# wangty537/raft_optical_flow

Hardware: AMD Instinct MI355X
Metric: image-pairs/s at Sintel 436x1024, 32 iters; corr-lookup GB/s vs HBM peak (higher is better)
Workload: dtype fp32 (convs: f16x3 split MFMA, fp32 accumulate); 1 GPU; RAFT-full inference, 436x1024 padded to 440x1024, 1 pair(s)/GPU/step, iters=32, all-pairs corr, hipGraph; global_batch=1, parallelism=frame-pair sharding x1

## Files before the change

include/raft_hip.h:

```cpp
#ifndef RAFT_HIP_H_
#define RAFT_HIP_H_

#include <stddef.h>

#ifdef __cplusplus
extern "C" {
#endif

#define RAFT_HIP_ABI_VERSION 19

#define RAFT_E_INVALID (-1)
#define RAFT_E_ALIGN (-2)

typedef void* raft_stream_t;

int raft_hip_abi_version(void);
const char* raft_hip_arch(void);
const char* raft_hip_last_error(void);
const char* raft_hip_source_hash(void);
int raft_debug_launch_span(int enable);
int raft_debug_launch_span_read(unsigned long long* host, int n);
int raft_debug_fill_lds_nan(raft_stream_t stream);

size_t raft_corr_pyramid_floats(int B, int H, int W, int num_levels);
// ... 82 lines not shown
typedef struct raft_conv2d_params {
  const float* in0; int in0_ld; int in0_c;
  const float* in1; int in1_ld; int in1_c;
  int batch, in_h, in_w;
  int out_h, out_w;
  int kh, kw, stride_h, stride_w, pad_h, pad_w;
  int mode;
  const float* weight;
  const float* bias;
  int n;
  float* out; int out_ld;
  int epilogue; float alpha; int split;
  const float* aux0; int aux0_ld;
  const float* aux1; int aux1_ld;
  float* out1; int out1_ld;
  const float* add0; int add0_ld;
  int precision;
  int* range_flag;
  float* stats_part; int stats_ld;
  const float* in_norm; int in_norm_relu;
  const void* weight_s;
} raft_conv2d_params;

#define RAFT_RANGE_LIMIT 32768.0f

int raft_conv2d_stats_slots(const raft_conv2d_params* p);
int raft_conv2d_halo_tile_rows(const raft_conv2d_params* p);
int raft_conv2d_halo_tiles_per_wg(const raft_conv2d_params* p);
#define RAFT_CONV_KERNEL_HALO 1
#define RAFT_CONV_KERNEL_GEMM 2
#define RAFT_CONV_KERNEL_STEM 3
#define RAFT_CONV_KERNEL_SMALLN 4
#define RAFT_CONV_KERNEL_SMALLN3X3 5
struct raft_conv2d_form {
  int kernel;
  int tile_rows;
  int tile_cols;
  int tiles_per_wg;
  int loader_waves;
  int compute_waves_per_simd;
  int gemm_k_groups;
  int smalln_tile_rows;
};
int raft_conv2d_form(const raft_conv2d_params* p, struct raft_conv2d_form* out);
int raft_conv2d_pair_form(const raft_conv2d_params* p0, const raft_conv2d_params* p1,
                          struct raft_conv2d_form out[2], int* one_launch);
int raft_conv2d_in_norm_ok(const raft_conv2d_params* p);
int raft_instnorm_merge(const float* part, int slots_per_image, int B, int C, int stats_ld, float eps,
                        float* stats, raft_stream_t stream);
size_t raft_instnorm_merge_ws_floats(int slots_per_image, int B, int C);
int raft_instnorm_merge_ws(const float* part, int slots_per_image, int B, int C, int stats_ld, float eps, void* ws,
                           float* stats, raft_stream_t stream);
size_t raft_instnorm_merge_counters(int B, int C);
int raft_instnorm_merge_fused(const float* part, int slots_per_image, int B, int C, int stats_ld, float eps, void* ws,
                              int* counters, float* stats, raft_stream_t stream);

int raft_conv2d_packed_shape(int mode, int n, int kh, int kw, int cin, int* n_pad, int* k_pad);
int raft_conv2d(const raft_conv2d_params* p, raft_stream_t stream);
int raft_conv2d_pair(const raft_conv2d_params* p0, const raft_conv2d_params* p1, raft_stream_t stream);
int raft_conv2d_set_halo_loaders(int nl);
int raft_conv2d_set_halo_ks(int ks);
int raft_conv2d_split_weight(const float* w, void* out, int n_pad, int k_pad, raft_stream_t stream);
size_t raft_conv2d_split_scaled_bytes(int n_pad, int k_pad);
int raft_conv2d_split_weight_scaled(const float* w, void* out, int n_pad, int k_pad, raft_stream_t stream);
int raft_conv2d_split_weight_prec(const float* w, void* out, int n_pad, int k_pad, int precision,
                                  raft_stream_t stream);
// ... 69 lines not shown
```

raft_optical_flow_amd/_lib.py:

```python
from __future__ import annotations

import ctypes
import os
import threading

_HERE = os.path.dirname(os.path.abspath(__file__))
LIB_PATH = os.environ.get("RAFT_HIP_LIB") or os.path.join(_HERE, "libraft_hip.so")

c_int = ctypes.c_int
c_float = ctypes.c_float
c_size_t = ctypes.c_size_t
c_long = ctypes.c_long
c_void_p = ctypes.c_void_p
c_char_p = ctypes.c_char_p
P = c_void_p

RAFT_CONV_VEC = 0
RAFT_CONV_GATHER = 1

PREC_FP32 = 0
PREC_F16X3 = 1
PREC_F16 = 2
PREC_BF16 = 3
PRECISIONS = {"fp32": PREC_FP32, "f16x3": PREC_F16X3, "f16": PREC_F16, "bf16": PREC_BF16}
# ... 25 lines not shown
        ("batch", c_int), ("in_h", c_int), ("in_w", c_int),
        ("out_h", c_int), ("out_w", c_int),
        ("kh", c_int), ("kw", c_int), ("stride_h", c_int), ("stride_w", c_int), ("pad_h", c_int), ("pad_w", c_int),
        ("mode", c_int),
        ("weight", P), ("bias", P),
        ("n", c_int),
        ("out", P), ("out_ld", c_int),
        ("epilogue", c_int), ("alpha", c_float), ("split", c_int),
        ("aux0", P), ("aux0_ld", c_int),
        ("aux1", P), ("aux1_ld", c_int),
        ("out1", P), ("out1_ld", c_int),
        ("add0", P), ("add0_ld", c_int),
        ("precision", c_int),
        ("range_flag", P),
        ("stats_part", P), ("stats_ld", c_int),
        ("in_norm", P), ("in_norm_relu", c_int),
        ("weight_s", P),
    ]


CARRY_MAX_SEGS = 8


class Copy2D(ctypes.Structure):

    _fields_ = [("src", P), ("src_ld", c_long), ("dst", P), ("dst_ld", c_long), ("rows", c_long), ("cols", c_long)]


CONV_KERNEL_HALO = 1
CONV_KERNEL_GEMM = 2
CONV_KERNEL_STEM = 3
CONV_KERNEL_SMALLN = 4
CONV_KERNEL_SMALLN3X3 = 5


class ConvForm(ctypes.Structure):

    _fields_ = [
        ("kernel", c_int), ("tile_rows", c_int), ("tile_cols", c_int), ("tiles_per_wg", c_int),
        ("loader_waves", c_int), ("compute_waves_per_simd", c_int), ("gemm_k_groups", c_int),
        ("smalln_tile_rows", c_int),
    ]

    def astuple(self):
        return tuple(getattr(self, f) for f, _ in self._fields_)


def conv_form(p: ConvParams) -> ConvForm:
    f = ConvForm()
    call("raft_conv2d_form", ctypes.byref(p), ctypes.byref(f))
    return f


def conv_pair_form(p0: ConvParams, p1: ConvParams):
    f = (ConvForm * 2)()
    one = c_int(0)
    call("raft_conv2d_pair_form", ctypes.byref(p0), ctypes.byref(p1), f, ctypes.byref(one))
    return f[0], f[1], bool(one.value)


_PROTOS = {
    "raft_hip_abi_version": (c_int, []),
    "raft_hip_arch": (c_char_p, []),
    "raft_hip_last_error": (c_char_p, []),
    "raft_hip_source_hash": (c_char_p, []),
    "raft_debug_fill_lds_nan": (c_int, [P]),
# ... 151 lines not shown
```

raft_optical_flow_amd/csrc/conv_halo.hip:

```cpp
#include <atomic>
#include <type_traits>

#include "conv_common.hpp"

namespace raft {
namespace {

constexpr int HTW = 16;
constexpr int HTH = 8;
constexpr int HTH_BIG = 16;
constexpr int HALO_LDS = 160 * 1024;

struct HaloArgs {
  raft_conv2d_params p;
  const float* inv_scale;
  int K;
  int nch;
  int nk;
  int gn;
  int tx_n, ty_n;
  unsigned w_bytes, in0_bytes, in1_bytes;
};

struct HaloLaunch {
  HaloArgs a[2];
  int sp0, sp1;
  int m;
  int grid0;
};

constexpr int patch_slots(int T, int U, int D, int late = 0) {
  for (int pa = 1; pa < 16; ++pa) {
    bool ok = true;
    for (int c = pa; c < 512 && ok; ++c) {
      const int last = (c - pa) * T + T - 1;
      const int rd = last == 0 ? -1 : (last - 1) / U;
      ok = (c * T) / U - D > rd + late;
    }
    if (ok) return pa;
  }
  return 16;
}
constexpr int halo_lds_bytes(int T, int U, int D, int BNT, int PI, int WR) {
  return U * (D + 1) * BNT * WR + patch_slots(T, U, D) * PI * 1024;
}

template <int KH, int KW, int BNT, int WR = 128, int TH = HTH>
struct HaloCfg {
  static constexpr int T = KH * KW;
  static constexpr int U = (BNT == 32 && T > 1) ? 4 : 2;
  static constexpr int LB = HALO_LDS;
  static constexpr int PH = TH + KH - 1, PW = HTW + KW - 1, NPIX = PH * PW;
  static constexpr int PI = (NPIX + 7) / 8;
#ifdef HALO_D
  static constexpr int D = halo_lds_bytes(T, U, HALO_D, BNT, PI, WR) <= LB   ? HALO_D
                           : halo_lds_bytes(T, U, 3, BNT, PI, WR) <= LB ? 3
                                                                              : 2;
#else
  static constexpr int D = halo_lds_bytes(T, U, 3, BNT, PI, WR) <= LB ? 3 : 2;
#endif
  static constexpr int PA = patch_slots(T, U, D);
#ifndef HALO_WX
#define HALO_WX 0
#endif
  static constexpr int DW = (T > 1 && D == 3 && HALO_WX > 0 &&
                             U * (D + HALO_WX + 1) * BNT * WR + PA * PI * 1024 + 16 * 1024 <= LB)
                                ? D + HALO_WX
                                : D;
  static constexpr int SB = U * (DW + 1);
  static constexpr int LDS_B = SB * BNT * WR, LDS_A = PA * PI * 1024;
};

#ifdef STAMPS
__device__ unsigned long long g_hstamp[8 * 16384];
__device__ unsigned long long g_lstamp[8 * 16384];
__device__ __forceinline__ unsigned long long hstamp_real() {
  unsigned long long t;
  __builtin_amdgcn_sched_barrier(0);
  asm volatile("s_memrealtime %0\n\ts_waitcnt lgkmcnt(0)" : "=s"(t)::"memory");
  __builtin_amdgcn_sched_barrier(0);
  return t;
}
__device__ __forceinline__ unsigned long long hstamp_now() {
  unsigned long long t;
  __builtin_amdgcn_sched_barrier(0);
  asm volatile("s_memtime %0\n\ts_waitcnt lgkmcnt(0)" : "=s"(t)::"memory");
  __builtin_amdgcn_sched_barrier(0);
  return t;
}
#endif

constexpr int gcd_c(int a, int b) { return b == 0 ? a : gcd_c(b, a % b); }
__host__ __device__ inline int halo_nkp(int nk, int U, int T, bool multi) {
  const int l = multi ? U / gcd_c(U, T) * T : U;
  return cdiv(nk, l) * l;
}
template <int KH, int KW, int BNT, int PREC, bool ENC>
constexpr int halo_norm_bytes(int LDS_B, int LDS_A, int D) {
  return (ENC && KH == 3 && KW == 3 && D == 3) ? ((HALO_LDS - LDS_B - LDS_A) & ~1023) : 0;
}

template <int KH, int KW, int BNT, int PREC, bool ENC = false, int TH = HTH, bool MT = false, int NL = 4, int KS = 1>
__device__ __forceinline__ void halo_body(const HaloArgs* args, int prob, int nt, int st0, int ntl_arg, char* smem) {
  constexpr bool X3 = PREC == RAFT_PREC_F16X3;
  constexpr bool BF = PREC == RAFT_PREC_BF16;
  using C = HaloCfg<KH, KW, BNT, X3 ? 128 : 64, TH>;
  constexpr int T = C::T, U = C::U, D = C::D, PW = C::PW, NPIX = C::NPIX, PI = C::PI, PA = C::PA, SB = C::SB;
  constexpr int DW = C::DW;
  constexpr int WROW = X3 ? 128 : 64;
  constexpr int QPR = WROW / 16;
  constexpr int RPP = 1024 / WROW;
  constexpr int NBI = BNT / RPP;
  constexpr int NWP = U * NBI / NL;
#ifndef HALO_KSW
#define HALO_KSW 0
#endif
  constexpr bool KSW = KS > 1 && HALO_KSW;
  constexpr int NWPC = KSW ? U * NBI / (4 * KS) : 1;
  constexpr int LNWP = KSW ? 0 : NWP;
  constexpr int WN = BNT == 128 ? 2 : 1;
  constexpr int WVM = 4 / WN;
  constexpr int MF = TH / 2 / WVM;
  constexpr int WCOL = BNT / WN;
  constexpr int NSUB = WCOL / 32;
  constexpr bool SC = X3 && TH == HTH_BIG;
  static_assert(MF >= 1 && MF * WVM * 2 == TH, "tile rows");
  static_assert(!(X3 && MF > 1) || SC, "f16x3 2 x 2 blocks need the one-accumulator (scaled) form");
  static_assert(!ENC || WN == 1, "the InstanceNorm partials are per 32-pixel block of all columns");

#ifndef HALO_NOLSPLIT
#define HALO_NOLSPLIT 0
#endif
  constexpr bool LSPLIT = T > 1 && D == 3 && !(HALO_NOLSPLIT && !ENC);
#ifndef HALO_SGB
#define HALO_SGB 1
#endif
  constexpr int SGB = (ENC && NL == 8) ? 0 : HALO_SGB;
#ifndef HALO_RELAX
#define HALO_RELAX 1
#endif
  constexpr int NRD1 = NSUB * 2 * (X3 ? 2 : 1) + MF * 2 * (X3 ? 2 : 1);
  constexpr bool RELAX = HALO_RELAX && SGB > 0 && LSPLIT && !MT && patch_slots(T, U, D, 1) == PA && NRD1 <= 15;
  static_assert(D >= 2 && C::LDS_B + C::LDS_A <= C::LB, "LDS budget");
  static_assert(KS == 1 || (KS == 2 && !MT && !ENC && LSPLIT && SGB > 0 && MF == 1 && NSUB <= 2 && (NL == 4 || NL == 8) &&
                            SB % 2 == 0 && 8 * 4096 <= C::LDS_B + C::LDS_A && (DW == D || !KSW) && NBI % NWPC == 0 &&
                            NWPC >= 1),
                "the K-split form: one tile of 32 x 64 blocks on the pre-split path, 4 loaders");
  static_assert(NWP >= 1 && NBI % NWP == 0, "a wave's weight pieces lie in one K-step");
  static_assert(U % 2 == 0 && (T == 1 || T >= U), "fragment parity; at most one chunk start per load set");
  constexpr int NORM_BYTES = halo_norm_bytes<KH, KW, BNT, PREC, ENC>(C::LDS_B, C::LDS_A, D);
  static_assert(NORM_BYTES == 0 || NORM_BYTES >= 256 * 8, "room for one image's norm table");

#ifdef STAMPS
  const unsigned long long r_entry = hstamp_real(), c_entry = hstamp_now();
#endif
  const int lane = threadIdx.x & 63;
  const int w = __builtin_amdgcn_readfirstlane(threadIdx.x >> 6);
  constexpr int NCW = 4 * KS;
  const bool loader = w >= NCW;
  const int lw = loader ? w - NCW : w;
  const int wc = w & 3;
  const int kp = KS > 1 ? (w >> 2) & (KS - 1) : 0;

  const HaloArgs& a = args[prob];
  const raft_conv2d_params& p = a.p;
  const int per = a.tx_n * a.ty_n;
  struct Tile {
    int b, y0, x0, n0, st;
  };
  auto tile_calc = [&](int k) {
    Tile t;
    t.st = st0 + k;
    t.b = t.st / per;
    const int sr = t.st - t.b * per;
    t.y0 = (sr / a.tx_n) * TH;
    t.x0 = (sr % a.tx_n) * HTW;
    t.n0 = nt * BNT;
    return t;
  };
  const Tile tile0 = tile_calc(0);
  auto tile_at = [&](int k) { return MT ? tile_calc(k) : tile0; };
  const int ntl = MT ? ntl_arg : 1;
  const int nk = a.nk, nch = a.nch;
// ... 62 lines not shown
    const bool in = j < nk && (!MT || kt < ntl);
    const int c = j / T, t = j - c * T;
    const int n0 = MT && in ? nt * BNT : 0;
    const unsigned soff = in ? (unsigned)(t * nch + c) * 128u + (unsigned)n0 * ((unsigned)a.K * 4u) : 0u;
    char* dst = smem + (U * (u % (DW + 1)) + q.ew) * (BNT * WROW) + q.wpc0 * 1024;
#pragma unroll
    for (int k = 0; k < NWP; ++k) dma16(rs_w, dst + k * 1024, in ? q.off[k] : OFF_INVALID, soff);
  };
  auto issue_weights = [&](int u) { issue_weights_q(u, wp0); };

  float* norm_tab = reinterpret_cast<float*>(smem + C::LDS_B + C::LDS_A);
  int b_first = 0;
  if constexpr (NORM_BYTES > 0) {
    if (p.in_norm) {
      b_first = tile_at(0).b;
      const int nb = tile_at(ntl - 1).b - b_first + 1;
      if (loader)
        for (int i = 64 * lw + lane; i < nb * 2 * p.in0_c; i += 64 * NL)
          norm_tab[i] = p.in_norm[(long)b_first * 2 * p.in0_c + i];
      __syncthreads();
    }
  }

  if (loader) {
#ifdef HALO_LPRIO
    __builtin_amdgcn_s_setprio(HALO_LPRIO);
#endif
    const __amdgpu_buffer_rsrc_t rs0 = make_rsrc(p.in0, a.in0_bytes);
    const __amdgpu_buffer_rsrc_t rs1 = make_rsrc(p.in1_c ? p.in1 : p.in0, p.in1_c ? a.in1_bytes : a.in0_bytes);
    const int in0_c = p.in0_c, in1_c = p.in1_c;
    const unsigned ld0 = p.in0_ld, ld1 = p.in1_c ? p.in1_ld : p.in0_ld;
    const int in_h = p.in_h, in_w = p.in_w;
    auto patch_pix = [&](const Tile& t, int pp) -> unsigned {
      const int py = pp / PW, px = pp - py * PW;
      const int iy = t.y0 + py - (KH - 1) / 2, ix = t.x0 + px - (KW - 1) / 2;
      const bool ok = pp < NPIX && (unsigned)iy < (unsigned)in_h && (unsigned)ix < (unsigned)in_w;
      return ok ? (unsigned)t.b * (unsigned)(in_h * in_w) + (unsigned)iy * (unsigned)in_w + (unsigned)ix : OFF_INVALID;
    };
    auto set_chunk = [&](int u, int& kt, int& c) -> bool {
      int ul;
      set_tile(u, kt, ul);
      c = (U * ul + T - 1) / T;
      return (!MT || kt < ntl) && c * T < U * ul + U;
    };
    constexpr int PK = (PI + NL - 1) / NL;
    const int pcw = PI > lw ? (PI - 1 - lw) / NL + 1 : 0;
    unsigned pq4[PK], ppix0[PK];
#pragma unroll
    for (int k = 0; k < PK; ++k) {
      const int pp = 8 * (lw + NL * k) + (lane >> 3);
      pq4[k] = 4u * (unsigned)((lane & 7) ^ (((pp % PW) >> 1) & 7));
      ppix0[k] = MT ? 0u : patch_pix(tile0, pp);
    }
    auto issue_patch = [&](int kt, int c) {
      const Tile t = tile_at(kt);
      const bool s0 = 32 * c < in0_c;
      const unsigned cb = (unsigned)(s0 ? 32 * c : 32 * c - in0_c);
      const unsigned lim = (unsigned)(s0 ? in0_c : in1_c);
      const unsigned ld = s0 ? ld0 : ld1;
      char* base = smem + C::LDS_B + pslot(kt, c) * (PI * 1024);
#pragma unroll
      for (int k = 0; k < PK; ++k) {
        if (lw + NL * k < PI) {
          const unsigned pix = MT ? patch_pix(t, 8 * (lw + NL * k) + (lane >> 3)) : ppix0[k];
          const unsigned ch = cb + pq4[k];
          const unsigned voff = (pix != OFF_INVALID && ch < lim) ? (pix * ld + ch) * 4u : OFF_INVALID;
          dma16(s0 ? rs0 : rs1, base + (lw + NL * k) * 1024, voff, 0);
        }
      }
    };
    auto issue_set = [&](int u, bool weights) -> int {
      int n = 0;
      if (weights) {
        issue_weights(u);
        n = NWP;
      }
      if constexpr (T == 1) {
        int kt, ul;
        set_tile(u, kt, ul);
        if (MT && kt >= ntl) return n;
#pragma unroll
        for (int e = 0; e < U; ++e) issue_patch(kt, U * ul + e);
        return n + U * pcw;
      } else {
        int kt, c;
        if (set_chunk(u, kt, c)) {
          issue_patch(kt, c);
          return n + pcw;
        }
        return n;
      }
    };
    if constexpr (LSPLIT) {
      constexpr int NT = 4 * NPIX, TI = (NT + 64 * NL - 1) / (64 * NL);
      const unsigned tg8 = 8u * (unsigned)(lane & 3);
      int tlds[TI];
      unsigned tpix0[TI];
#pragma unroll
      for (int i = 0; i < TI; ++i) {
        const int t = 64 * lw + lane + 64 * NL * i;
        const int pp = t >> 2, g = t & 3;
        const int px = pp % PW;
        tlds[i] = t < NT ? pp * 128 + ((g ^ ((px >> 1) & 7)) << 4) : -1;
        tpix0[i] = MT ? 0u : patch_pix(tile0, pp);
      }
      auto task_pix = [&](const Tile& tt, int i) {
        return MT ? patch_pix(tt, (64 * lw + lane + 64 * NL * i) >> 2) : tpix0[i];
      };
      using Staged = f32x4[TI][2];
      auto load_patch = [&](int kt, int c, Staged& dst) {
        const Tile tt = tile_at(kt);
        const bool s0 = 32 * c < in0_c;
        const unsigned cb = (unsigned)(s0 ? 32 * c : 32 * c - in0_c);
        const unsigned lim = (unsigned)(s0 ? in0_c : in1_c);
        const unsigned ld = s0 ? ld0 : ld1;
#pragma unroll
        for (int i = 0; i < TI; ++i) {
          const unsigned pix = task_pix(tt, i);
#pragma unroll
          for (int q = 0; q < 2; ++q) {
            const unsigned ch = cb + tg8 + 4u * q;
            const unsigned voff = (pix != OFF_INVALID && ch < lim) ? (pix * ld + ch) * 4u : OFF_INVALID;
            dst[i][q] = buf_load4<0>(s0 ? rs0 : rs1, voff, 0);
          }
        }
      };
      const bool nrm = NORM_BYTES > 0 && p.in_norm != nullptr;
      auto store_patch = [&](int kt, int c, const Staged& src) {
        char* base = smem + C::LDS_B + pslot(kt, c) * (PI * 1024);
        const bool s0 = 32 * c < in0_c;
        if (nrm && s0) {
          const Tile tt = tile_at(kt);
          const float2* tab = reinterpret_cast<const float2*>(norm_tab) + (tt.b - b_first) * in0_c;
#pragma unroll
          for (int i = 0; i < TI; ++i) {
// ... 126 lines not shown
#endif
          }
        }
        if constexpr (DW > D && !KSW) {
          if (s + DW < NS) {
            issue_weights(s + DW);
            nnew += NWP;
          }
        }
        LSTAMP(l_w);
        wait_vm_n(s + 1 < NS ? nnew + (DW - D) * NWP : 0);
        __builtin_amdgcn_s_waitcnt(0xC07F);
        LSTAMP(l_wait);
        __builtin_amdgcn_s_barrier();
        LSTAMP(l_bar);
      }
#undef LSTAMP
#ifdef STAMPS
      {
        const unsigned lid = blockIdx.x * NL + lw;
        if (lane == 0 && lid < 16384) {
          unsigned long long* g = g_lstamp + lid * 8;
          g[0] = l_st;
          g[1] = l_ld;
          g[2] = l_w;
          g[3] = l_wait;
          g[4] = l_bar;
          g[5] = hstamp_now() - l_loop;
          g[6] = 1;
        }
      }
#endif
      wait_vm<0>();
      if constexpr (KS > 1) __builtin_amdgcn_s_barrier();
      return;
    }
    constexpr int NH = D > 3 ? D - 3 : 1;
    int hist[NH];
    {
      int cnt[D];
#pragma unroll
      for (int u = 0; u < D; ++u) cnt[u] = issue_set(u, false);
      int n = 0;
#pragma unroll
      for (int u = 2; u < D; ++u) n += cnt[u];
      wait_vm_n(n);
#pragma unroll
      for (int k = 0; k < NH; ++k) hist[k] = k < D - 3 ? cnt[D - 1 - k] : 0;
    }
    __builtin_amdgcn_s_barrier();
    for (int s = 0; s < NS; ++s) {
      const int nnew = s + D < NS ? issue_set(s + D, true) : 0;
      int n = D >= 3 ? nnew : 0;
#pragma unroll
      for (int k = 0; k < D - 3; ++k) n += hist[k];
      wait_vm_n(s + 1 < NS ? n : 0);
      __builtin_amdgcn_s_barrier();
#pragma unroll
      for (int k = NH - 1; k > 0; --k) hist[k] = hist[k - 1];
      hist[0] = nnew;
    }
    wait_vm<0>();
    return;
  }

  const int m = lane & 31, h = lane >> 5;
  const int wm = wc % WVM, cb = (wc / WVM) * WCOL;
  int ppbase[MF];
#pragma unroll
  for (int f = 0; f < MF; ++f) ppbase[f] = (2 * (wm * MF + f) + (m >> 4)) * PW + (m & 15);
  const int bsw = X3 ? (m >> 1) & 7 : (m >> 2) & 3;
  constexpr int AXF = X3 && !SC ? MF : 1, AXS = X3 && !SC ? NSUB : 1;
  f32x16 acc[MF][NSUB], accx[AXF][AXS];
  auto clear_acc = [&]() {
#pragma unroll
    for (int f = 0; f < MF; ++f)
#pragma unroll
      for (int sb = 0; sb < NSUB; ++sb) acc[f][sb] = f32x16{};
#pragma unroll
    for (int f = 0; f < AXF; ++f)
#pragma unroll
      for (int sb = 0; sb < AXS; ++sb) accx[f][sb] = f32x16{};
  };
  clear_acc();
  int b_bs = kp;
  int a_t = 0, a_ky = 0, a_kx = 0, a_ps = 0;
  struct Frag {
    h8 ah[MF][2], al[MF][2];
    h8 bh[NSUB][2], bl[NSUB][2];
  };
  f32x4 av[MF][4];
  auto read_b = [&](Frag& F) {
    const char* Bb = smem + b_bs * (BNT * WROW);
#pragma unroll
    for (int sb = 0; sb < NSUB; ++sb) {
#pragma unroll
      for (int qq = 0; qq < 2; ++qq) {
        F.bh[sb][qq] = *reinterpret_cast<const h8*>(Bb + (cb + sb * 32 + m) * WROW + (((2 * h + qq) ^ bsw) << 4));
        if constexpr (X3)
          F.bl[sb][qq] = *reinterpret_cast<const h8*>(Bb + (cb + sb * 32 + m) * WROW + (((4 + 2 * h + qq) ^ bsw) << 4));
      }
    }
    b_bs = b_bs + KS >= SB ? b_bs + KS - SB : b_bs + KS;
  };
  auto advance_a = [&]() {
    ++a_kx;
    if (a_kx == KW) {
      a_kx = 0;
      ++a_ky;
    }
    if (++a_t == T) {
      a_t = 0;
      a_ky = 0;
      a_ps = a_ps + 1 == PA ? 0 : a_ps + 1;
    }
  };
  auto read_a = [&]() {
    const char* Ab = smem + C::LDS_B + a_ps * (PI * 1024);
    const int sw = (((m & 15) + a_kx) >> 1) & 7;
#pragma unroll
    for (int f = 0; f < MF; ++f) {
      const int pp = ppbase[f] + (a_ky * PW + a_kx);
#pragma unroll
      for (int jq = 0; jq < 4; ++jq)
        av[f][jq] = *reinterpret_cast<const f32x4*>(Ab + pp * 128 + (((4 * h + jq) ^ sw) << 4));
    }
    advance_a();
  };
  auto read_a_split = [&](Frag& F) {
    const char* Ab = smem + C::LDS_B + a_ps * (PI * 1024);
    const int sw = (((m & 15) + a_kx) >> 1) & 7;
#pragma unroll
    for (int f = 0; f < MF; ++f) {
      const char* row = Ab + (ppbase[f] + (a_ky * PW + a_kx)) * 128;
#pragma unroll
      for (int qq = 0; qq < 2; ++qq) {
        F.ah[f][qq] = *reinterpret_cast<const h8*>(row + (((2 * h + qq) ^ sw) << 4));
        if constexpr (X3) F.al[f][qq] = *reinterpret_cast<const h8*>(row + (((4 + 2 * h + qq) ^ sw) << 4));
      }
    }
#pragma unroll
    for (int k = 0; k < KS; ++k) advance_a();
  };
  auto split_a = [&](Frag& F) {
#pragma unroll
    for (int f = 0; f < MF; ++f) {
#ifdef HALO_ABL_NOSPLIT
      F.ah[f][0] = __builtin_bit_cast(h8, av[f][0]);
      F.al[f][0] = __builtin_bit_cast(h8, av[f][1]);
      F.ah[f][1] = __builtin_bit_cast(h8, av[f][2]);
      F.al[f][1] = __builtin_bit_cast(h8, av[f][3]);
#else
      split8<X3, BF>(av[f][0], av[f][1], F.ah[f][0], F.al[f][0]);
      split8<X3, BF>(av[f][2], av[f][3], F.ah[f][1], F.al[f][1]);
#endif
    }
  };
  auto mfma_step = [&](const Frag& F) {
#pragma unroll
    for (int qq = 0; qq < 2; ++qq) {
      if constexpr (BF) {
#pragma unroll
        for (int f = 0; f < MF; ++f)
#pragma unroll
          for (int sb = 0; sb < NSUB; ++sb)
            acc[f][sb] = __builtin_amdgcn_mfma_f32_32x32x16_bf16(
                __builtin_bit_cast(bf8, F.ah[f][qq]), __builtin_bit_cast(bf8, F.bh[sb][qq]), acc[f][sb], 0, 0, 0);
// ... 43 lines not shown
  };
  auto epilogue = [&](const Tile& t) {
    if constexpr (SC) {
#pragma unroll
      for (int sb = 0; sb < NSUB; ++sb) {
        const float is = a.inv_scale[t.n0 + cb + sb * 32 + m];
#pragma unroll
        for (int f = 0; f < MF; ++f)
#pragma unroll
          for (int r = 0; r < 16; ++r) acc[f][sb][r] *= is;
      }
    } else if constexpr (X3) {
#pragma unroll
      for (int f = 0; f < MF; ++f)
#pragma unroll
        for (int sb = 0; sb < NSUB; ++sb)
#pragma unroll
          for (int r = 0; r < 16; ++r) acc[f][sb][r] += accx[f][sb][r] * (1.0f / SPLIT_SCALE);
    }
    f32x4 stv[NSUB];
    const int oh = __builtin_amdgcn_readfirstlane(p.out_h), ow = __builtin_amdgcn_readfirstlane(p.out_w);
    const int rowb = t.b * oh;
#pragma unroll
    for (int f = 0; f < MF; ++f) {
      int rows[16];
#pragma unroll
      for (int r = 0; r < 16; ++r) {
        const int mm = (r & 3) + 8 * (r >> 2) + 4 * h;
        const int y = t.y0 + 2 * (wm * MF + f) + (mm >> 4), x = t.x0 + (mm & 15);
        rows[r] = ((y < oh) & (x < ow)) ? (rowb + y) * ow + x : -1;
      }
#pragma unroll
      for (int sb = 0; sb < NSUB; ++sb) tile_epilogue<false>(p, rows, t.n0 + cb + sb * 32 + m, acc[f][sb]);
      if constexpr (ENC) {
        if (p.stats_part) {
#pragma unroll
          for (int sb = 0; sb < NSUB; ++sb) {
            const int n = t.n0 + sb * 32 + m;
            const f32x4 v = tile_stats_vals(rows, acc[f][sb], p.bias ? p.bias[n < p.n ? n : 0] : 0.f);
            stv[sb] = f == 0 ? v : stats_combine(stv[sb], v);
            if (f == MF - 1) stats_write(p, n, (long)t.st * 4 + w, stv[sb]);
          }
        }
      }
    }
  };

  auto epilogue_ks2 = [&](const Tile& t) {
    if constexpr (KS > 1 && NSUB == 1) {
      if constexpr (X3 && !SC) {
#pragma unroll
        for (int r = 0; r < 16; ++r) acc[0][0][r] += accx[0][0][r] * (1.0f / SPLIT_SCALE);
      }
      f32x4* mine = reinterpret_cast<f32x4*>(smem + (wc * 2 + kp) * 4096) + lane * 2;
      const f32x4* theirs = reinterpret_cast<const f32x4*>(smem + (wc * 2 + (kp ^ 1)) * 4096) + lane * 2;
#pragma unroll
      for (int q = 0; q < 2; ++q) {
        f32x4 v;
#pragma unroll
        for (int i = 0; i < 4; ++i) v[i] = kp ? acc[0][0][4 * q + i] : acc[0][0][8 + 4 * q + i];
        mine[q ^ (lane & 1)] = v;
      }
      __builtin_amdgcn_s_waitcnt(0xC07F);
      __builtin_amdgcn_s_barrier();
      f32x16 keep = acc[0][0];
#pragma unroll
      for (int q = 0; q < 2; ++q) {
// ... 240 lines not shown
    if constexpr (LSPLIT) {
      read_b(F[0]);
      read_a_split(F[0]);
    } else {
      read_b(F[0]);
      split_a(F[0]);
      read_a();
    }
#ifdef STAMPS
    const unsigned long long t4 = hstamp_now();
    t_epi += t4 - t0;
    t0 = t4;
#endif
  }
  }
#ifdef STAMPS
  {
    const unsigned long long c_exit = hstamp_now(), r_exit = hstamp_real();
    const unsigned wid = blockIdx.x * NCW + w;
    if (lane == 0 && wid < 16384) {
      unsigned long long* g = g_hstamp + wid * 8;
      g[0] = r_entry;
      g[1] = r_exit;
      g[2] = c_loop - c_entry;
      g[3] = t_cmp;
      g[4] = t_wait + t_bar;
      g[5] = t_epi;
      g[6] = c_exit - c_entry;
    }
  }
#endif
}

template <int KH, int KW, int BNT, int PREC, bool ENC = false, int TH = HTH, bool MT = false, int NL = 4, int KS = 1>
__global__ __launch_bounds__(64 * (4 * KS + NL)) void conv_halo_kernel(HaloLaunch hl) {
  using C = HaloCfg<KH, KW, BNT, PREC == RAFT_PREC_F16X3 ? 128 : 64, TH>;
  constexpr int NORM_BYTES = halo_norm_bytes<KH, KW, BNT, PREC, ENC>(C::LDS_B, C::LDS_A, C::D);
  __shared__ __attribute__((aligned(1024))) char smem[C::LDS_B + C::LDS_A + NORM_BYTES];
  int g = xcd_tile(blockIdx.x, gridDim.x);
  const int prob = g >= hl.grid0 ? 1 : 0;
  g -= prob * hl.grid0;
  const int gn = hl.a[prob].gn;
  if constexpr (MT) {
    const int st0 = (g / gn) * hl.m;
    const int ntl = min(hl.m, (prob ? hl.sp1 : hl.sp0) - st0);
    halo_body<KH, KW, BNT, PREC, ENC, TH, true, NL>(hl.a, prob, g % gn, st0, ntl, smem);
  } else {
    halo_body<KH, KW, BNT, PREC, ENC, TH, false, NL, KS>(hl.a, prob, g % gn, g / gn, 1, smem);
  }
}

std::atomic<int> g_halo_nl{0};
bool halo_nl8() {
  int v = g_halo_nl.load(std::memory_order_relaxed);
  if (v == 0) {
    const char* e = getenv("RAFT_HALO_NL8");
    v = e && e[0] == '0' ? 4 : 8;
    g_halo_nl.store(v, std::memory_order_relaxed);
  }
  return v == 8;
}
#ifndef HALO_KS2_NL8
#define HALO_KS2_NL8 0
#endif
#ifndef HALO_KS2_BN32
#define HALO_KS2_BN32 0
#endif
std::atomic<int> g_halo_ks{0};
bool halo_ks2() {
  int v = g_halo_ks.load(std::memory_order_relaxed);
  if (v == 0) {
    const char* e = getenv("RAFT_HALO_KS2");
    v = e && e[0] == '0' ? 1 : 2;
    g_halo_ks.store(v, std::memory_order_relaxed);
  }
  return v == 2;
}
bool halo_nl8_enc() {
  const char* e = getenv("RAFT_HALO_NL8_ENC");
  return !(e && e[0] == '0');
}
constexpr bool halo_no_mt(int prec, int taps, int bn) { return prec != RAFT_PREC_F16X3 && taps == 9 && bn == 128; }

template <int KH, int KW, int BNT, int PREC, bool ENC, int TH, bool MT, int NL = 4, int KS = 1>
void halo_start(const HaloLaunch& l, dim3 grid, hipStream_t s, ConvForm* q) {
  if (q) {
    *q = ConvForm{};
    q->kernel = RAFT_CONV_KERNEL_HALO;
    q->tile_rows = TH;
    q->tile_cols = BNT;
    q->tiles_per_wg = MT ? l.m : 1;
    q->loader_waves = NL;
    q->compute_waves_per_simd = KS;
    return;
  }
  hipLaunchKernelGGL((conv_halo_kernel<KH, KW, BNT, PREC, ENC, TH, MT, NL, KS>), grid, dim3(64 * (4 * KS + NL)), 0, s, l);
}

template <int KH, int KW, int BNT, int PREC, bool ENC = false, int TH = HTH>
void launch_halo_mt(const HaloLaunch& l, dim3 grid, hipStream_t s, ConvForm* q) {
  constexpr bool NO_MT = halo_no_mt(PREC, KH * KW, BNT);
  if (NO_MT && l.m > 1) {
    fprintf(stderr, "raft_hip: internal error: a one-tile-only halo conv was planned with %d tiles per work-group\n", l.m);
    abort();
  }
  constexpr bool CAN_NL8 = PREC == RAFT_PREC_F16X3 && !ENC && TH == HTH && BNT <= 64 && KH * KW > 1;
  constexpr bool CAN_NL8E = PREC == RAFT_PREC_F16X3 && ENC && TH == HTH && BNT <= 64 && KH * KW == 9;
  if constexpr (CAN_NL8E) {
    if (halo_nl8_enc()) {
      if (l.m > 1)
        halo_start<KH, KW, BNT, PREC, ENC, TH, true, 8>(l, grid, s, q);
      else
        halo_start<KH, KW, BNT, PREC, ENC, TH, false, 8>(l, grid, s, q);
      return;
    }
  }
  constexpr bool CAN_KS2 = CAN_NL8 && (BNT == 64 || (BNT == 32 && HALO_KS2_BN32)) &&
                           HaloCfg<KH, KW, BNT, 128, TH>::D == 3 && !HALO_NOLSPLIT;
  if (!NO_MT && l.m > 1) {
    halo_start<KH, KW, BNT, PREC, ENC, TH, !NO_MT>(l, grid, s, q);
  } else {
    if constexpr (CAN_KS2) {
      if (halo_ks2()) {
#if HALO_KS2_NL8
        halo_start<KH, KW, BNT, PREC, ENC, TH, false, 8, 2>(l, grid, s, q);
#else
        halo_start<KH, KW, BNT, PREC, ENC, TH, false, 4, 2>(l, grid, s, q);
#endif
        return;
// ... 219 lines not shown
  l.m = (int)m;
  l.sp0 = (int)s0;
  l.sp1 = (int)s1;
  l.grid0 = (int)(g0 * cdiv_l(s0, m));
  if (cost_out) *cost_out = best;
  return wgs(m);
}

double halo_mt_plan_cost(const HaloOperands& o, int th) {
  HaloLaunch l;
  if (!halo_problem(o, l.a[0])) return 1e30;
  halo_set_th(o, l.a[0], th);
  const int bn = th == HTH_BIG ? 64 : halo_spatial(l.a[0]) * (o.n_pad / 64) > 128 ? 64 : 32;
  l.a[0].gn = o.n_pad / bn;
  l.a[1] = l.a[0];
  double cost = 1e30;
  halo_plan_grid(l, bn, th, false, &cost);
  return cost;
}

void launch_halo(const HaloLaunch& l, int bn, int th, long wgs, hipStream_t s, ConvForm* q) {
  const raft_conv2d_params& p = l.a[0].p;
  dim3 grid((unsigned)wgs);
  if (p.kh == 1 && p.kw == 1)
    launch_halo_k<1, 1>(l, bn, th, grid, s, q);
  else if (p.kh == 3)
    launch_halo_k<3, 3>(l, bn, th, grid, s, q);
  else if (p.kh == 1)
    launch_halo_k<1, 5>(l, bn, th, grid, s, q);
  else
    launch_halo_k<5, 1>(l, bn, th, grid, s, q);
}


}

#ifdef STAMPS
extern "C" int raft_debug_hstamps(unsigned long long* host, int n) {
  return (int)hipMemcpyFromSymbol(host, HIP_SYMBOL(g_hstamp), sizeof(unsigned long long) * (size_t)n);
}
extern "C" int raft_debug_lstamps(unsigned long long* host, int n, int clear) {
  if (clear) {
    static unsigned long long zero[8 * 16384];
    return (int)hipMemcpyToSymbol(HIP_SYMBOL(g_lstamp), zero, sizeof(zero));
  }
  return (int)hipMemcpyFromSymbol(host, HIP_SYMBOL(g_lstamp), sizeof(unsigned long long) * (size_t)n);
}
#endif

extern "C" int raft_conv2d_set_halo_loaders(int nl) {
  const int prev = halo_nl8() ? 8 : 4;
  if (nl == 4 || nl == 8) g_halo_nl.store(nl, std::memory_order_relaxed);
  return prev;
}

extern "C" int raft_conv2d_set_halo_ks(int ks) {
  const int prev = halo_ks2() ? 2 : 1;
  if (ks == 1 || ks == 2) g_halo_ks.store(ks, std::memory_order_relaxed);
  return prev;
}

bool conv_halo_norm_ok(const HaloOperands& o) {
  HaloArgs a;
  if (!halo_enabled() || !halo_problem(o, a)) return false;
  const raft_conv2d_params& p = o.p;
  return p.kh == 3 && p.kw == 3 && p.in0_c <= 256 && HaloCfg<3, 3, 64>::D == 3 && HaloCfg<3, 3, 32>::D == 3;
}

long halo_wide_min() {
  static const long v = [] {
    const char* e = getenv("RAFT_HALO_WIDE_MIN");
    return e ? atol(e) : 256L;
  }();
  return v;
}
bool halo_wide_enabled() {
  static const bool enabled = [] {
    const char* e = getenv("RAFT_HALO_WIDE");
    return !(e && e[0] == '0');
  }();
  return enabled;
}

int halo_pick(const HaloOperands& o, const HaloArgs& a, bool& wide) {
  const raft_conv2d_params& p = o.p;
  const bool can = p.precision != RAFT_PREC_F16X3 && !p.stats_part && !p.in_norm && o.n_pad % 128 == 0 &&
                   halo_wide_enabled();
  const long n = halo_spatial(a) * (o.n_pad / 128);
  wide = can && n >= 512;
  const int th = halo_pick_th(o, wide);
  if (!wide && th != HTH_BIG) wide = can && n >= halo_wide_min();
  return th;
}

int conv_halo_tile_rows(const HaloOperands& o) {
  HaloArgs a;
  if (!halo_enabled() || !halo_problem(o, a)) return 0;
  bool wide;
  return halo_pick(o, a, wide);
}

bool conv_halo_covers(const HaloOperands& o) {
  HaloArgs a;
  return halo_enabled() && halo_problem(o, a);
}

int conv_halo_stats_slots(const HaloOperands& o) {
  HaloArgs a;
  if (!halo_enabled() || !halo_problem(o, a)) return 0;
  if (!((o.p.kh == 1 && o.p.kw == 1) || (o.p.kh == 3 && o.p.kw == 3))) return 0;
  const int th = halo_pick_th(o, false);
  return a.tx_n * cdiv(o.p.out_h, th) * 4;
}

static bool halo_plan(const HaloOperands& o, HaloLaunch& l, int& bn, int& th, long& wgs) {
  if (!halo_enabled() || !halo_problem(o, l.a[0])) return false;
  const long spatial = halo_spatial(l.a[0]);
  bool wide;
  th = halo_pick(o, l.a[0], wide);
  bn = th == HTH_BIG ? 64 : wide ? 128 : spatial * (o.n_pad / 64) > 128 ? 64 : 32;
  halo_set_th(o, l.a[0], th);
  l.a[0].gn = o.n_pad / bn;
  const long tiles = halo_spatial(l.a[0]) * l.a[0].gn;
  if (tiles >= (1L << 31)) return false;
  l.a[1] = l.a[0];
  wgs = halo_plan_grid(l, bn, th, false);
  return true;
}

int conv_halo_tiles_per_wg(const HaloOperands& o) {
  HaloLaunch l;
  int bn, th;
  long wgs;
  return halo_plan(o, l, bn, th, wgs) ? l.m : 0;
}

int conv_halo_launch(const HaloOperands& o, hipStream_t s, ConvForm* q) {
  HaloLaunch l;
  int bn, th;
  long wgs;
  if (!halo_plan(o, l, bn, th, wgs)) return 1;
  launch_halo(l, bn, th, wgs, s, q);
  return 0;
}

int conv_halo_launch_pair(const HaloOperands& o0, const HaloOperands& o1, hipStream_t s, ConvForm* q) {
  HaloLaunch l;
  if (!halo_enabled() || !halo_problem(o0, l.a[0]) || !halo_problem(o1, l.a[1])) return 1;
  const raft_conv2d_params &p0 = o0.p, &p1 = o1.p;
  if (p0.kh != p1.kh || p0.kw != p1.kw || p0.precision != p1.precision) return 1;
  const int th = halo_pick_th(o0, false);
  if (halo_pick_th(o1, false) != th) return 1;
  halo_set_th(o0, l.a[0], th);
  halo_set_th(o1, l.a[1], th);
  const long s0 = halo_spatial(l.a[0]), s1 = halo_spatial(l.a[1]);
  const int bn = th == HTH_BIG ? 64 : s0 * (o0.n_pad / 64) + s1 * (o1.n_pad / 64) > 128 ? 64 : 32;
  if (o0.n_pad % bn || o1.n_pad % bn) return 1;
  l.a[0].gn = o0.n_pad / bn;
  l.a[1].gn = o1.n_pad / bn;
  const long t0 = s0 * l.a[0].gn, tiles = t0 + s1 * l.a[1].gn;
  if (tiles >= (1L << 31)) return 1;
  launch_halo(l, bn, th, halo_plan_grid(l, bn, th, true), s, q);
  if (q) q[1] = q[0];
  return 0;
}


}
```

Baseline: 141.3 image-pairs/s.

## Add stride-2 halo conv path with parity-plane LDS patches

Adds a stride-2 variant of the halo convolution kernel for 3x3 pad-1 (and, opt-in, 1x1) convs. Input patches are stored in LDS as four even/odd row/column parity planes, so each stride-2 tap reads a contiguous plane with the existing swizzled MFMA fragment loads. It also adds an InstanceNorm stats path that combines the two 32-pixel blocks per work-group through LDS with an extra barrier. It is enabled by default only for small grids, at most one work-group per CU, and is meant to replace the slower generic/GEMM path used for the encoder's downsampling convs. The cost is more template instantiations and extra index arithmetic in the loader and A-fragment reads.

```diff
diff --git a/include/raft_hip.h b/include/raft_hip.h
--- a/include/raft_hip.h
+++ b/include/raft_hip.h
@@ -138,6 +138,7 @@
 #define RAFT_CONV_KERNEL_STEM 3
 #define RAFT_CONV_KERNEL_SMALLN 4
 #define RAFT_CONV_KERNEL_SMALLN3X3 5
+#define RAFT_CONV_KERNEL_HALO_S2 6
 struct raft_conv2d_form {
   int kernel;
   int tile_rows;
diff --git a/raft_optical_flow_amd/_lib.py b/raft_optical_flow_amd/_lib.py
--- a/raft_optical_flow_amd/_lib.py
+++ b/raft_optical_flow_amd/_lib.py
@@ -81,6 +81,7 @@
 CONV_KERNEL_STEM = 3
 CONV_KERNEL_SMALLN = 4
 CONV_KERNEL_SMALLN3X3 = 5
+CONV_KERNEL_HALO_S2 = 6
 
 
 class ConvForm(ctypes.Structure):
diff --git a/raft_optical_flow_amd/csrc/conv_halo.hip b/raft_optical_flow_amd/csrc/conv_halo.hip
--- a/raft_optical_flow_amd/csrc/conv_halo.hip
+++ b/raft_optical_flow_amd/csrc/conv_halo.hip
@@ -45,12 +45,38 @@
   return U * (D + 1) * BNT * WR + patch_slots(T, U, D) * PI * 1024;
 }
 
-template <int KH, int KW, int BNT, int WR = 128, int TH = HTH>
+constexpr int HTH_S2 = 4;
+template <int TH>
+struct S2Planes {
+  static constexpr int W0 = HTW + 2, W1 = HTW, H0 = TH + 1, H1 = TH;
+  static constexpr int B00 = 0, B01 = H0 * W0, B10 = H0 * (W0 + W1), B11 = B10 + H1 * W0;
+  static constexpr int NPIX = B11 + H1 * W1;
+  static_assert(B01 % 2 == 0 && B10 % 2 == 0 && B11 % 2 == 0, "even plane bases");
+};
+template <int TH>
+__device__ __forceinline__ void s2_plane_pix(int pp, int& pr, int& pc, int& i, int& j) {
+  using P = S2Planes<TH>;
+  pr = pp >= P::B10 ? 1 : 0;
+  const int q0 = pp - (pr ? P::B10 : 0);
+  const int n0 = (pr ? P::H1 : P::H0) * P::W0;
+  pc = q0 >= n0 ? 1 : 0;
+  const int q = q0 - (pc ? n0 : 0), pw = pc ? P::W1 : P::W0;
+  i = q / pw;
+  j = q - i * pw;
+}
+template <int TH>
+__device__ __forceinline__ int s2_plane_base(int pr, int pc) {
+  using P = S2Planes<TH>;
+  return pr ? (pc ? P::B11 : P::B10) : (pc ? P::B01 : P::B00);
+}
+
+template <int KH, int KW, int BNT, int WR = 128, int TH = HTH, int S = 1>
 struct HaloCfg {
   static constexpr int T = KH * KW;
   static constexpr int U = (BNT == 32 && T > 1) ? 4 : 2;
   static constexpr int LB = HALO_LDS;
-  static constexpr int PH = TH + KH - 1, PW = HTW + KW - 1, NPIX = PH * PW;
+  static constexpr int PH = TH + KH - 1, PW = HTW + KW - 1;
+  static constexpr int NPIX = (S == 2 && T > 1) ? S2Planes<TH>::NPIX : PH * PW;
   static constexpr int PI = (NPIX + 7) / 8;
 #ifdef HALO_D
   static constexpr int D = halo_lds_bytes(T, U, HALO_D, BNT, PI, WR) <= LB   ? HALO_D
@@ -95,17 +121,21 @@
   const int l = multi ? U / gcd_c(U, T) * T : U;
   return cdiv(nk, l) * l;
 }
-template <int KH, int KW, int BNT, int PREC, bool ENC>
+template <int KH, int KW, int BNT, int PREC, bool ENC, int S = 1>
 constexpr int halo_norm_bytes(int LDS_B, int LDS_A, int D) {
-  return (ENC && KH == 3 && KW == 3 && D == 3) ? ((HALO_LDS - LDS_B - LDS_A) & ~1023) : 0;
-}
-
-template <int KH, int KW, int BNT, int PREC, bool ENC = false, int TH = HTH, bool MT = false, int NL = 4, int KS = 1>
+  return (ENC && KH == 3 && KW == 3 && D == 3 && S == 1) ? ((HALO_LDS - LDS_B - LDS_A) & ~1023) : 0;
+}
+
+template <int KH, int KW, int BNT, int PREC, bool ENC = false, int TH = HTH, bool MT = false, int NL = 4, int KS = 1,
+          int S = 1>
 __device__ __forceinline__ void halo_body(const HaloArgs* args, int prob, int nt, int st0, int ntl_arg, char* smem) {
   constexpr bool X3 = PREC == RAFT_PREC_F16X3;
   constexpr bool BF = PREC == RAFT_PREC_BF16;
-  using C = HaloCfg<KH, KW, BNT, X3 ? 128 : 64, TH>;
+  using C = HaloCfg<KH, KW, BNT, X3 ? 128 : 64, TH, S>;
   constexpr int T = C::T, U = C::U, D = C::D, PW = C::PW, NPIX = C::NPIX, PI = C::PI, PA = C::PA, SB = C::SB;
+  constexpr bool S2P = S == 2 && T > 1;
+  static_assert(S == 1 || (S == 2 && TH == HTH_S2 && BNT == 64 && !MT && KS == 1 && NL == 4 && (T == 1 || T == 9)),
+                "the stride-2 form: 4 x 16-pixel x 64-column tiles, one per work-group");
   constexpr int DW = C::DW;
   constexpr int WROW = X3 ? 128 : 64;
   constexpr int QPR = WROW / 16;
@@ -118,7 +148,7 @@
   constexpr bool KSW = KS > 1 && HALO_KSW;
   constexpr int NWPC = KSW ? U * NBI / (4 * KS) : 1;
   constexpr int LNWP = KSW ? 0 : NWP;
-  constexpr int WN = BNT == 128 ? 2 : 1;
+  constexpr int WN = (BNT == 128 || TH == HTH_S2) ? 2 : 1;
   constexpr int WVM = 4 / WN;
   constexpr int MF = TH / 2 / WVM;
   constexpr int WCOL = BNT / WN;
@@ -126,12 +156,13 @@
   constexpr bool SC = X3 && TH == HTH_BIG;
   static_assert(MF >= 1 && MF * WVM * 2 == TH, "tile rows");
   static_assert(!(X3 && MF > 1) || SC, "f16x3 2 x 2 blocks need the one-accumulator (scaled) form");
-  static_assert(!ENC || WN == 1, "the InstanceNorm partials are per 32-pixel block of all columns");
+  static_assert(!ENC || WN == 1 || S == 2, "the InstanceNorm partials are per 32-pixel block of all columns");
 
 #ifndef HALO_NOLSPLIT
 #define HALO_NOLSPLIT 0
 #endif
-  constexpr bool LSPLIT = T > 1 && D == 3 && !(HALO_NOLSPLIT && !ENC);
+  constexpr bool LSPLIT = T > 1 && D == 3 && (S2P || !(HALO_NOLSPLIT && !ENC));
+  static_assert(!S2P || LSPLIT, "the parity planes are written by the loaders' split stores");
 #ifndef HALO_SGB
 #define HALO_SGB 1
 #endif
@@ -148,7 +179,7 @@
                 "the K-split form: one tile of 32 x 64 blocks on the pre-split path, 4 loaders");
   static_assert(NWP >= 1 && NBI % NWP == 0, "a wave's weight pieces lie in one K-step");
   static_assert(U % 2 == 0 && (T == 1 || T >= U), "fragment parity; at most one chunk start per load set");
-  constexpr int NORM_BYTES = halo_norm_bytes<KH, KW, BNT, PREC, ENC>(C::LDS_B, C::LDS_A, D);
+  constexpr int NORM_BYTES = halo_norm_bytes<KH, KW, BNT, PREC, ENC, S>(C::LDS_B, C::LDS_A, D);
   static_assert(NORM_BYTES == 0 || NORM_BYTES >= 256 * 8, "room for one image's norm table");
 
 #ifdef STAMPS
@@ -277,9 +308,25 @@
     const unsigned ld0 = p.in0_ld, ld1 = p.in1_c ? p.in1_ld : p.in0_ld;
     const int in_h = p.in_h, in_w = p.in_w;
     auto patch_pix = [&](const Tile& t, int pp) -> unsigned {
-      const int py = pp / PW, px = pp - py * PW;
-      const int iy = t.y0 + py - (KH - 1) / 2, ix = t.x0 + px - (KW - 1) / 2;
-      const bool ok = pp < NPIX && (unsigned)iy < (unsigned)in_h && (unsigned)ix < (unsigned)in_w;
+      int iy, ix;
+      bool in = pp < NPIX;
+      if constexpr (S2P) {
+        int i, j, pr, pc;
+        s2_plane_pix<TH>(pp, pr, pc, i, j);
+        const int px = 2 * j + pc;
+        in = in && px <= 2 * HTW;
+        iy = 2 * t.y0 - 1 + 2 * i + pr;
+        ix = 2 * t.x0 - 1 + px;
+      } else if constexpr (S == 2) {
+        const int py = pp / PW, px = pp - py * PW;
+        iy = 2 * (t.y0 + py);
+        ix = 2 * (t.x0 + px);
+      } else {
+        const int py = pp / PW, px = pp - py * PW;
+        iy = t.y0 + py - (KH - 1) / 2;
+        ix = t.x0 + px - (KW - 1) / 2;
+      }
+      const bool ok = in && (unsigned)iy < (unsigned)in_h && (unsigned)ix < (unsigned)in_w;
       return ok ? (unsigned)t.b * (unsigned)(in_h * in_w) + (unsigned)iy * (unsigned)in_w + (unsigned)ix : OFF_INVALID;
     };
     auto set_chunk = [&](int u, int& kt, int& c) -> bool {
@@ -345,7 +392,11 @@
       for (int i = 0; i < TI; ++i) {
         const int t = 64 * lw + lane + 64 * NL * i;
         const int pp = t >> 2, g = t & 3;
-        const int px = pp % PW;
+        int px = pp % PW;
+        if constexpr (S2P) {
+          int pr, pc, pi;
+          s2_plane_pix<TH>(pp < NPIX ? pp : 0, pr, pc, pi, px);
+        }
         tlds[i] = t < NT ? pp * 128 + ((g ^ ((px >> 1) & 7)) << 4) : -1;
         tpix0[i] = MT ? 0u : patch_pix(tile0, pp);
       }
@@ -538,7 +589,7 @@
       }
 #endif
       wait_vm<0>();
-      if constexpr (KS > 1) __builtin_amdgcn_s_barrier();
+      if constexpr (KS > 1 || (ENC && S == 2)) __builtin_amdgcn_s_barrier();
       return;
     }
     constexpr int NH = D > 3 ? D - 3 : 1;
@@ -567,6 +618,7 @@
       hist[0] = nnew;
     }
     wait_vm<0>();
+    if constexpr (ENC && S == 2) __builtin_amdgcn_s_barrier();
     return;
   }
 
@@ -574,7 +626,7 @@
   const int wm = wc % WVM, cb = (wc / WVM) * WCOL;
   int ppbase[MF];
 #pragma unroll
-  for (int f = 0; f < MF; ++f) ppbase[f] = (2 * (wm * MF + f) + (m >> 4)) * PW + (m & 15);
+  for (int f = 0; f < MF; ++f) ppbase[f] = (2 * (wm * MF + f) + (m >> 4)) * (S2P ? 16 : PW) + (m & 15);
   const int bsw = X3 ? (m >> 1) & 7 : (m >> 2) & 3;
   constexpr int AXF = X3 && !SC ? MF : 1, AXS = X3 && !SC ? NSUB : 1;
   f32x16 acc[MF][NSUB], accx[AXF][AXS];
@@ -635,10 +687,17 @@
   };
   auto read_a_split = [&](Frag& F) {
     const char* Ab = smem + C::LDS_B + a_ps * (PI * 1024);
-    const int sw = (((m & 15) + a_kx) >> 1) & 7;
+    const int ox = S2P ? a_kx >> 1 : a_kx;
+    const int sw = (((m & 15) + ox) >> 1) & 7;
+    int tap_off = a_ky * PW + a_kx, tap_pw = PW;
+    if constexpr (S2P) {
+      tap_pw = (a_kx & 1) ? S2Planes<TH>::W1 : S2Planes<TH>::W0;
+      tap_off = s2_plane_base<TH>(a_ky & 1, a_kx & 1) + (a_ky >> 1) * tap_pw + ox;
+    }
 #pragma unroll
     for (int f = 0; f < MF; ++f) {
-      const char* row = Ab + (ppbase[f] + (a_ky * PW + a_kx)) * 128;
+      const int pp = S2P ? (ppbase[f] >> 4) * tap_pw + (ppbase[f] & 15) + tap_off : ppbase[f] + tap_off;
+      const char* row = Ab + pp * 128;
 #pragma unroll
       for (int qq = 0; qq < 2; ++qq) {
         F.ah[f][qq] = *reinterpret_cast<const h8*>(row + (((2 * h + qq) ^ sw) << 4));
@@ -748,7 +807,24 @@
       }
 #pragma unroll
       for (int sb = 0; sb < NSUB; ++sb) tile_epilogue<false>(p, rows, t.n0 + cb + sb * 32 + m, acc[f][sb]);
-      if constexpr (ENC) {
+      if constexpr (ENC && S == 2) {
+        static_assert(MF == 1 && NSUB == 1 && WVM == 2, "two 32-pixel blocks x two 32-column halves");
+        const bool on = p.stats_part != nullptr;
+        const int n = t.n0 + cb + m;
+        f32x4 v{};
+        if (on) v = tile_stats_vals(rows, acc[0][0], p.bias ? p.bias[n < p.n ? n : 0] : 0.f);
+        f32x4* xch = reinterpret_cast<f32x4*>(smem) + cb + m;
+        if (wm == 1 && h == 0) *xch = v;
+        __builtin_amdgcn_s_waitcnt(0xC07F);
+        __builtin_amdgcn_s_barrier();
+        if (on && wm == 0) {
+          v = stats_combine(v, *xch);
+          const int slots = 2 * cdiv(oh * ow, 64);
+          const int sr = t.st - t.b * per;
+          stats_write(p, n, (long)t.b * slots + sr, v);
+          if (per + sr < slots) stats_write(p, n, (long)t.b * slots + per + sr, f32x4{});
+        }
+      } else if constexpr (ENC) {
         if (p.stats_part) {
 #pragma unroll
           for (int sb = 0; sb < NSUB; ++sb) {
@@ -1055,10 +1131,11 @@
 #endif
 }
 
-template <int KH, int KW, int BNT, int PREC, bool ENC = false, int TH = HTH, bool MT = false, int NL = 4, int KS = 1>
+template <int KH, int KW, int BNT, int PREC, bool ENC = false, int TH = HTH, bool MT = false, int NL = 4, int KS = 1,
+          int S = 1>
 __global__ __launch_bounds__(64 * (4 * KS + NL)) void conv_halo_kernel(HaloLaunch hl) {
-  using C = HaloCfg<KH, KW, BNT, PREC == RAFT_PREC_F16X3 ? 128 : 64, TH>;
-  constexpr int NORM_BYTES = halo_norm_bytes<KH, KW, BNT, PREC, ENC>(C::LDS_B, C::LDS_A, C::D);
+  using C = HaloCfg<KH, KW, BNT, PREC == RAFT_PREC_F16X3 ? 128 : 64, TH, S>;
+  constexpr int NORM_BYTES = halo_norm_bytes<KH, KW, BNT, PREC, ENC, S>(C::LDS_B, C::LDS_A, C::D);
   __shared__ __attribute__((aligned(1024))) char smem[C::LDS_B + C::LDS_A + NORM_BYTES];
   int g = xcd_tile(blockIdx.x, gridDim.x);
   const int prob = g >= hl.grid0 ? 1 : 0;
@@ -1069,7 +1146,7 @@
     const int ntl = min(hl.m, (prob ? hl.sp1 : hl.sp0) - st0);
     halo_body<KH, KW, BNT, PREC, ENC, TH, true, NL>(hl.a, prob, g % gn, st0, ntl, smem);
   } else {
-    halo_body<KH, KW, BNT, PREC, ENC, TH, false, NL, KS>(hl.a, prob, g % gn, g / gn, 1, smem);
+    halo_body<KH, KW, BNT, PREC, ENC, TH, false, NL, KS, S>(hl.a, prob, g % gn, g / gn, 1, smem);
   }
 }
 
@@ -1105,11 +1182,11 @@
 }
 constexpr bool halo_no_mt(int prec, int taps, int bn) { return prec != RAFT_PREC_F16X3 && taps == 9 && bn == 128; }
 
-template <int KH, int KW, int BNT, int PREC, bool ENC, int TH, bool MT, int NL = 4, int KS = 1>
+template <int KH, int KW, int BNT, int PREC, bool ENC, int TH, bool MT, int NL = 4, int KS = 1, int S = 1>
 void halo_start(const HaloLaunch& l, dim3 grid, hipStream_t s, ConvForm* q) {
   if (q) {
     *q = ConvForm{};
-    q->kernel = RAFT_CONV_KERNEL_HALO;
+    q->kernel = S == 2 ? RAFT_CONV_KERNEL_HALO_S2 : RAFT_CONV_KERNEL_HALO;
     q->tile_rows = TH;
     q->tile_cols = BNT;
     q->tiles_per_wg = MT ? l.m : 1;
@@ -1117,7 +1194,7 @@
     q->compute_waves_per_simd = KS;
     return;
   }
-  hipLaunchKernelGGL((conv_halo_kernel<KH, KW, BNT, PREC, ENC, TH, MT, NL, KS>), grid, dim3(64 * (4 * KS + NL)), 0, s, l);
+  hipLaunchKernelGGL((conv_halo_kernel<KH, KW, BNT, PREC, ENC, TH, MT, NL, KS, S>), grid, dim3(64 * (4 * KS + NL)), 0, s, l);
 }
 
 template <int KH, int KW, int BNT, int PREC, bool ENC = false, int TH = HTH>
@@ -1403,6 +1480,77 @@
     launch_halo_k<5, 1>(l, bn, th, grid, s, q);
 }
 
+bool halo_s2_enabled() {
+  const char* e = getenv("RAFT_HALO_S2");
+  return !(e && e[0] == '0');
+}
+int halo_s2_slots(const raft_conv2d_params& p) { return 2 * cdiv(p.out_h * p.out_w, 64); }
+constexpr long HALO_S2_MIN_TILES = 4;
+bool halo_problem_s2(const HaloOperands& o, HaloArgs& a) {
+  const raft_conv2d_params& p = o.p;
+  if (!halo_s2_enabled() || p.mode != RAFT_CONV_VEC || p.stride_h != 2 || p.stride_w != 2) return false;
+  if (p.precision != RAFT_PREC_F16X3 && p.precision != RAFT_PREC_F16 && p.precision != RAFT_PREC_BF16) return false;
+  const bool k3 = p.kh == 3 && p.kw == 3 && p.pad_h == 1 && p.pad_w == 1;
+  const bool k1 = p.kh == 1 && p.kw == 1 && p.pad_h == 0 && p.pad_w == 0;
+  if (!k3 && !k1) return false;
+  if (k1) {
+    const char* e = getenv("RAFT_HALO_S2_1X1");
+    if (!(e && e[0] == '1')) return false;
+  }
+  if (p.n <= 4 || p.in1_c != 0 || p.in0_c % 32 != 0 || p.in_norm || o.n_pad % 64 != 0) return false;
+  a.p = p;
+  a.inv_scale = nullptr;
+  a.K = o.k_pad;
+  a.nch = o.k_pad / (p.kh * p.kw) / 32;
+  a.nk = a.nch * p.kh * p.kw;
+  a.tx_n = cdiv(p.out_w, HTW);
+  a.ty_n = cdiv(p.out_h, HTH_S2);
+  a.w_bytes = o.w_bytes;
+  a.in0_bytes = o.in0_bytes;
+  a.in1_bytes = o.in1_bytes;
+  a.gn = o.n_pad / 64;
+  const long per = (long)a.tx_n * a.ty_n;
+  if (per * p.batch < HALO_S2_MIN_TILES) return false;
+  static const long max_wgs = [] {
+    const char* e = getenv("RAFT_HALO_S2_MAX_WGS");
+    return e ? atol(e) : 0L;
+  }();
+  if (per * p.batch * a.gn > (max_wgs > 0 ? max_wgs : halo_cus())) return false;
+  return per <= halo_s2_slots(p);
+}
+template <int KH, int KW, int PREC>
+void launch_halo_s2_p(const HaloLaunch& l, dim3 grid, hipStream_t s, ConvForm* q) {
+  if (l.a[0].p.stats_part)
+    halo_start<KH, KW, 64, PREC, true, HTH_S2, false, 4, 1, 2>(l, grid, s, q);
+  else
+    halo_start<KH, KW, 64, PREC, false, HTH_S2, false, 4, 1, 2>(l, grid, s, q);
+}
+template <int KH, int KW>
+void launch_halo_s2_k(const HaloLaunch& l, dim3 grid, hipStream_t s, ConvForm* q) {
+  const int prec = l.a[0].p.precision;
+  if (prec == RAFT_PREC_F16X3)
+    launch_halo_s2_p<KH, KW, RAFT_PREC_F16X3>(l, grid, s, q);
+  else if (prec == RAFT_PREC_BF16)
+    launch_halo_s2_p<KH, KW, RAFT_PREC_BF16>(l, grid, s, q);
+  else
+    launch_halo_s2_p<KH, KW, RAFT_PREC_F16>(l, grid, s, q);
+}
+bool halo_s2_launch(const HaloOperands& o, hipStream_t s, ConvForm* q) {
+  HaloLaunch l;
+  if (!halo_enabled() || !halo_problem_s2(o, l.a[0])) return false;
+  l.a[1] = l.a[0];
+  l.sp0 = (int)halo_spatial(l.a[0]);
+  l.sp1 = 0;
+  l.m = 1;
+  l.grid0 = l.sp0 * l.a[0].gn;
+  const dim3 grid((unsigned)l.grid0);
+  if (o.p.kh == 3)
+    launch_halo_s2_k<3, 3>(l, grid, s, q);
+  else
+    launch_halo_s2_k<1, 1>(l, grid, s, q);
+  return true;
+}
+
 
 }
 
@@ -1466,6 +1614,7 @@
 
 int conv_halo_tile_rows(const HaloOperands& o) {
   HaloArgs a;
+  if (halo_enabled() && halo_problem_s2(o, a)) return HTH_S2;
   if (!halo_enabled() || !halo_problem(o, a)) return 0;
   bool wide;
   return halo_pick(o, a, wide);
@@ -1473,11 +1622,12 @@
 
 bool conv_halo_covers(const HaloOperands& o) {
   HaloArgs a;
-  return halo_enabled() && halo_problem(o, a);
+  return halo_enabled() && (halo_problem(o, a) || halo_problem_s2(o, a));
 }
 
 int conv_halo_stats_slots(const HaloOperands& o) {
   HaloArgs a;
+  if (halo_enabled() && halo_problem_s2(o, a)) return halo_s2_slots(o.p);
   if (!halo_enabled() || !halo_problem(o, a)) return 0;
   if (!((o.p.kh == 1 && o.p.kw == 1) || (o.p.kh == 3 && o.p.kw == 3))) return 0;
   const int th = halo_pick_th(o, false);
@@ -1503,6 +1653,7 @@
   HaloLaunch l;
   int bn, th;
   long wgs;
+  if (halo_enabled() && halo_problem_s2(o, l.a[0])) return 1;
   return halo_plan(o, l, bn, th, wgs) ? l.m : 0;
 }
 
@@ -1510,6 +1661,7 @@
   HaloLaunch l;
   int bn, th;
   long wgs;
+  if (halo_s2_launch(o, s, q)) return 0;
   if (!halo_plan(o, l, bn, th, wgs)) return 1;
   launch_halo(l, bn, th, wgs, s, q);
   return 0;
```

Result: no change. 141.3 image-pairs/s, median of 4 (+0.0%).
